# weiguangzhao/PBNet

Hardware: AMD Instinct MI355X
Metric: scenes/sec fwd+cluster (ScanNet ~150k pts/scene) (higher is better)
Workload: dtype bf16; 1 GPU; configs[1]: 1 scene, 161517 pts, 146038 voxels @2cm, 1 rotated copy, full PBNet.forward (MinkUNet34C + grouping + MinkUNet14A mask + MinkUNet34C score); scenes_in_flight_per_gpu=4, scene_seeds=2 (configs[1])

## Files before the change

### include/pbnet_hip.h

```cpp
#ifndef PBNET_HIP_H
#define PBNET_HIP_H

#include <stddef.h>
#include <stdint.h>

#ifdef __cplusplus
extern "C" {
#endif

typedef void* pbn_stream_t;

enum {
    PBN_OK = 0,
    PBN_ERR_ARG = -1,
    PBN_ERR_WORKSPACE = -2,
    PBN_ERR_HIP = -3,
    PBN_ERR_RANGE = -4,
    PBN_ERR_UNSUPPORTED = -5
};

enum { PBN_F32 = 0, PBN_BF16 = 1, PBN_F16 = 2 };

#define PBN_MAX_SCENES 8

// ... 25 lines not shown
                      int capacity, int32_t* unique_index, int32_t* inverse, int32_t* unique_coords, int32_t* n_unique,
                      void* workspace, size_t workspace_bytes, pbn_stream_t stream);

int pbn_coords_stride(const int32_t* fine_coords, const int32_t* n_fine_dev, int n_fine_max, int stride_out,
                      uint64_t* table_keys, int32_t* table_vals, int capacity, int32_t* coarse_coords,
                      int32_t* parent_row, int32_t* child_k, int32_t* nbr_down, int32_t* n_coarse, void* workspace,
                      size_t workspace_bytes, pbn_stream_t stream);

int pbn_kernel_map(const int32_t* out_coords, const int32_t* n_out_dev, int n_out_max, const int32_t* offsets,
                   int n_offsets, const uint64_t* table_keys, const int32_t* table_vals, int capacity, int32_t* nbr,
                   pbn_stream_t stream);

int pbn_kernel_map_cube(const int32_t* out_coords, const int32_t* n_out_dev, int n_out_max, int kernel_size,
                        int tensor_stride, int x_fastest, const uint64_t* table_keys, const int32_t* table_vals,
                        int capacity, int32_t* nbr, pbn_stream_t stream);

int pbn_up_table(const int32_t* parent_row, const int32_t* child_k, const int32_t* n_fine_dev, int n_fine_max,
                 int32_t* nbr_up, pbn_stream_t stream);

int pbn_spconv_forward(const void* in_feat, int ld_in, int n_in, const int32_t* nbr, int n_offsets, const int32_t* row_perm,
                       const int32_t* n_out_dev, int n_out, const void* w_packed, int vecs_per_offset, int n_steps,
                       int cout_padded, const float* scale, const float* shift, const void* residual, int ld_res,
                       int relu, void* out_feat, int ld_out, int dtype, int rows_per_wave, void* workspace,
                       size_t workspace_bytes, pbn_stream_t stream);

int pbn_spconv_forward_dual(const void* in_feat, int ld_in, int n_in, const int32_t* nbr, int n_offsets,
                            const int32_t* n_out_dev, int n_out, const void* w_packed, int vecs_per_offset, int n_steps,
                            int cout_padded, const float* scale, const float* shift, const void* residual, int ld_res,
                            int relu, void* out_feat, int ld_out, int dtype, int rows_per_wave, void* workspace,
                            size_t workspace_bytes, const void* in2_feat, int ld_in2, int n_in2, int vecs_second,
                            pbn_stream_t stream);

int pbn_spconv_family(int n_out, int n_offsets, int vecs_per_offset, int n_steps, int cout_padded, int dtype, int has_map);

int pbn_gather_rows(const void* in, int ld_in_bytes, const int64_t* idx, int n, int row_bytes, void* out,
                    int ld_out_bytes, pbn_stream_t stream);

size_t pbn_segment_pool_workspace_bytes(int n_seg, int channels);
int pbn_segment_pool(const void* feats, int ld, int channels, int dtype, const int32_t* seg_start, int n_seg,
                     float* out_max, float* out_avg, void* workspace, size_t workspace_bytes, pbn_stream_t stream);

int pbn_local_scene_rows(const int32_t* ent_row_start, const int32_t* ent_member_start, const int32_t* ent_scene,
                         const float* ent_weight, int n_ent, int n_rows, const int32_t* member_idx,
                         const int64_t* ins_ind, const float* xyz, float inv_voxel, const void* point_feat, int ld_feat,
                         int channels, const void* sem_score, int ld_sem, const int64_t* sem_pred, int dtype,
                         int64_t* point_idx, int64_t* row_scene, int32_t* coords, void* feat_out, int ld_out,
                         pbn_stream_t stream);
int pbn_gather_pad_rows(const void* in, int ld_in_bytes, int row_bytes, const int64_t* idx, int n, void* out,
                        int ld_out_bytes, pbn_stream_t stream);

int pbn_pack_weight(const float* src, int n_offsets, int dim_a, int dim_b, int flip, int transpose, int dtype,
                    int vecs_per_offset, int n_steps, int cout_padded, void* out, pbn_stream_t stream);

typedef struct pbn_pack_job {
    const float* src;
    void* out;
    int32_t n_offsets, dim_a, dim_b, flip, transpose, cin, cout, cin_p, cout_p, n_steps;
    int32_t reserved[2];
} pbn_pack_job;
int pbn_pack_weights_batch(const pbn_pack_job* jobs, int n_jobs, int max_vectors, int dtype, pbn_stream_t stream);

int pbn_gather_rulebook_rows(const void* in, int ld_in_bytes, int row_bytes, const int32_t* nbr, int n_offsets, int k0,
                             int kc, int n, void* out, pbn_stream_t stream);

size_t pbn_bn_workspace_bytes(int channels);
int pbn_bn_train_forward(const void* x, int ld_x, int n, int channels, int dtype, const float* weight, const float* bias,
// ... 400 lines not shown
```

### pbnet_amd/_native.py

```python
import ctypes
import os

import torch

_HERE = os.path.dirname(os.path.abspath(__file__))
LIB_PATH = os.environ.get("PBNET_HIP_LIB") or os.path.join(_HERE, "libpbnet_hip.so")

_lib = None

c_f32p = ctypes.c_void_p
c_i32p = ctypes.c_void_p
c_vp = ctypes.c_void_p
c_int = ctypes.c_int
c_float = ctypes.c_float
c_size = ctypes.c_size_t

c_i64 = ctypes.c_int64
c_i32 = ctypes.c_int32

DT = {torch.float32: 0, torch.bfloat16: 1, torch.float16: 2}


class CoordsLayout(ctypes.Structure):
    _fields_ = [("counts", c_i64), ("unique_index", c_i64), ("inverse", c_i64),
# ... 74 lines not shown


class ApOverlaps(ctypes.Structure):
    _fields_ = [("n", c_i32), ("_pad", c_i32), ("th", ctypes.c_double * AP_MAX_OVERLAPS)]


class PostBatchLayout(ctypes.Structure):
    _fields_ = [(k, c_i64) for k in ("masks", "counts", "prop_scene", "score", "rows", "pick_rows", "n_rows", "n_pick", "iou",
                                     "votes", "sp_label", "seg", "seg_refined", "counts2", "renumber", "total_bytes")]


SIGNATURES = {
    "pbn_version": (ctypes.c_char_p, []),
    "pbn_last_hip_error": (c_int, []),
    "pbn_cluster_workspace_bytes": (c_size, [c_int, c_int, c_int]),
    "pbn_binary_cluster": (c_int, [c_f32p, c_f32p, c_i32p, c_i32p, c_int, c_int, c_float, c_int, c_float, c_int, c_int,
                                   c_i32p, c_i32p, c_i32p, c_f32p, c_i32p, c_i32p, c_i32p, c_i32p, c_vp, c_size, c_vp]),
    "pbn_get_iou": (c_int, [c_i32p, c_i32p, c_vp, c_i32p, c_f32p, c_int, c_int, c_vp]),
    "pbn_cal_iou_and_masklabel": (c_int, [c_i32p, c_i32p, c_vp, c_i32p, c_f32p, c_int, c_int, c_f32p, c_f32p, c_int,
                                          c_vp]),
    "pbn_hash_capacity": (c_int, [c_int]),
    "pbn_coords_workspace_bytes": (c_size, [c_int]),
    "pbn_coords_unique": (c_int, [c_i32p, c_i32p, c_int, c_vp, c_i32p, c_int, c_i32p, c_i32p, c_i32p, c_i32p, c_vp,
                                  c_size, c_vp]),
    "pbn_coords_stride": (c_int, [c_i32p, c_i32p, c_int, c_int, c_vp, c_i32p, c_int, c_i32p, c_i32p, c_i32p, c_i32p,
                                  c_i32p, c_vp, c_size, c_vp]),
    "pbn_kernel_map": (c_int, [c_i32p, c_i32p, c_int, c_i32p, c_int, c_vp, c_i32p, c_int, c_i32p, c_vp]),
    "pbn_up_table": (c_int, [c_i32p, c_i32p, c_i32p, c_int, c_i32p, c_vp]),
    "pbn_spconv_forward": (c_int, [c_vp, c_int, c_int, c_i32p, c_int, c_i32p, c_i32p, c_int, c_vp, c_int, c_int, c_int,
                                   c_f32p, c_f32p, c_vp, c_int, c_int, c_vp, c_int, c_int, c_int, c_vp, c_size, c_vp]),
    "pbn_spconv_forward_dual": (c_int, [c_vp, c_int, c_int, c_i32p, c_int, c_i32p, c_int, c_vp, c_int, c_int, c_int, c_f32p, c_f32p,
                                        c_vp, c_int, c_int, c_vp, c_int, c_int, c_int, c_vp, c_size, c_vp, c_int, c_int, c_int, c_vp]),
    "pbn_spconv_family": (c_int, [c_int, c_int, c_int, c_int, c_int, c_int, c_int]),
    "pbn_spconv_wgrad_workspace_bytes": (c_size, [c_int, c_int, c_int]),
    "pbn_spconv_wgrad": (c_int, [c_vp, c_int, c_vp, c_int, c_int, c_vp, c_vp, c_i32p, c_i32p, c_int, c_int, c_int, c_int, c_int,
                                 c_f32p, c_vp, c_size, c_vp]),
    "pbn_spconv_wgrad_checked": (c_int, [c_vp, c_int, ctypes.c_longlong, c_vp, c_int, ctypes.c_longlong, c_int, c_vp, c_vp, c_i32p,
                                         c_i32p, c_int, c_int, c_int, c_int, c_int, c_int, c_f32p, c_vp, c_size, c_vp]),
    "pbn_spconv_wgrad_plan": (c_int, [c_int, c_int, c_int, c_int, c_int, c_int, c_int, c_int, c_int, c_int, c_size,
                                      ctypes.POINTER(WgradPlan)]),
    "pbn_gather_rows": (c_int, [c_vp, c_int, c_vp, c_int, c_int, c_vp, c_int, c_vp]),
    "pbn_segment_pool_workspace_bytes": (c_size, [c_int, c_int]),
    "pbn_segment_pool": (c_int, [c_vp, c_int, c_int, c_int, c_i32p, c_int, c_f32p, c_f32p, c_vp, c_size, c_vp]),
    "pbn_local_scene_rows": (c_int, [c_i32p, c_i32p, c_i32p, c_f32p, c_int, c_int, c_i32p, c_vp, c_f32p, c_float, c_vp,
                                     c_int, c_int, c_vp, c_int, c_vp, c_int, c_vp, c_vp, c_i32p, c_vp, c_int, c_vp]),
    "pbn_gather_pad_rows": (c_int, [c_vp, c_int, c_int, c_vp, c_int, c_vp, c_int, c_vp]),
    "pbn_mlp_rows": (c_int, [c_vp, c_int, c_int, c_vp, c_vp, c_int, c_f32p, c_f32p, c_f32p, c_f32p, c_int, c_f32p, c_f32p,
                             c_int, c_int, c_vp, c_int, c_int, c_vp]),
    "pbn_select_blocks": (c_int, [c_int]),
    "pbn_sem_argmax_table": (c_int, [c_vp, c_int, c_int, c_i32p, c_int, c_int, c_int, c_vp, c_vp, c_i32p, c_i32p, c_vp]),
    "pbn_select_points": (c_int, [c_vp, c_int, c_int, c_i32p, c_i32p, c_f32p, c_vp, c_int, c_int, c_vp, c_f32p, c_f32p,
                                  c_i32p, c_vp]),
    "pbn_mask_count": (c_int, [c_vp, c_int, c_float, c_vp, c_int, c_int, c_int, c_i32p, c_i32p, c_vp]),
    "pbn_proposal_rows": (c_int, [c_vp, c_int, c_float, c_vp, c_vp, c_int, c_i32p, c_i32p, c_f32p, c_float, c_float, c_vp,
                                  c_int, c_int, c_int, c_vp, c_vp, c_i32p, c_vp, c_vp]),
    "pbn_post_words": (c_int, [c_int]),
    "pbn_proposal_bitmask": (c_int, [c_vp, c_int, c_int, c_int, c_vp, c_i32p, c_vp]),
    "pbn_mask_iou": (c_int, [c_vp, c_i32p, c_int, c_int, c_i32p, c_f32p, c_vp]),
    "pbn_superpoint_refine": (c_int, [c_vp, c_i32p, c_int, c_int, c_vp, c_int, c_vp, c_i32p, c_vp, c_vp, c_vp, c_i32p,
                                      c_vp]),
    "pbn_bitmask_to_dense": (c_int, [c_vp, c_i32p, c_int, c_int, c_i32p, c_vp]),
    "pbn_post_max_proposals": (c_int, []),
    "pbn_post_select": (c_int, [c_f32p, c_i32p, c_int, c_float, c_int, c_i32p, c_i32p, c_i32p, c_vp]),
    "pbn_mask_iou_dev": (c_int, [c_vp, c_i32p, c_i32p, c_int, c_int, c_i32p, c_f32p, c_vp]),
    "pbn_post_nms": (c_int, [c_f32p, c_i32p, c_i32p, c_int, c_f32p, c_float, c_i32p, c_i32p, c_i32p, c_vp]),
    "pbn_superpoint_refine_dev": (c_int, [c_vp, c_i32p, c_i32p, c_int, c_int, c_vp, c_int, c_vp, c_i32p, c_vp, c_vp, c_vp, c_i32p,
# ... 177 lines not shown
```

### pbnet_amd/csrc/executor.hip

```cpp
#include <cstdlib>
#include "pbn_common.h"
#include "spconv_common.h"
#include "unet_plan.h"

using namespace pbn;

static inline size_t a256(size_t x) { return align_up(x, 256); }

extern "C" size_t pbn_coords_arena_bytes(int n, int want_k5, pbn_coords_layout* L) {
    if (n < 0 || !L) return 0;
    const size_t N = (size_t)(n > 0 ? n : 1);
    const int cap = pbn_hash_capacity(n);
    size_t off = 0;
    auto take = [&](size_t bytes) { size_t o = off; off = a256(off + bytes); return (int64_t)o; };
    L->counts = take(16 * sizeof(int));
    for (int l = 0; l < 5; ++l) { L->capacity[l] = cap; L->keys[l] = take((size_t)cap * 8); }
    for (int l = 0; l < 4; ++l) L->nbr_down[l] = take(N * 8 * 4);
    for (int l = 0; l < 5; ++l) L->vals[l] = take((size_t)cap * 4);
    const int64_t fill_end = (int64_t)off;
    (void)fill_end;
    L->unique_index = take(N * 4);
    L->inverse = take(N * 4);
    for (int l = 0; l < 5; ++l) {
        L->coords[l] = take(N * 16);
// ... 169 lines not shown
}

static NextWeights next_weights(const pbn_unet_op& q, int n_bufs, const MapTables& T, const int32_t* n_rows, const PlanArena& B,
                                int dtype, int mode) {
    if (!op_index_ok(q.in_buf, q.res_buf, q.out_buf, q.level_in, q.level_out, n_bufs) || !q.w) return {};
    const OpTables m = op_tables(q.map_kind, q.level_in, q.level_out, T);
    const ConvArgs nx = shape_args(n_rows[q.level_out], m.K, q.vpo, q.n_steps, q.cout_p, m.fwd != nullptr,
                                   (unsigned)((unsigned long long)q.n_steps * (q.cout_p / 16) * 1024ull),
                                   (unsigned)((unsigned long long)n_rows[q.level_in] * B.ld(q.in_buf) * esize(dtype)));
    LaunchDesc d;
    describe_launch(nx, dtype, &d);
    return {q.w, q.n_steps, q.cout_p / 16, d.wave_family ? d.nt : 0, (mode == 1 && d.wmajor) ? d.groups : 0};
}

static int unet_forward_impl(const pbn_unet_op* ops, int n_ops, const pbn_unet_buf* bufs, int n_bufs,
                             const int32_t* n_rows, const void* input, int ld_input, const int32_t* const* k3,
                             const int32_t* k5, const int32_t* const* down, const int32_t* const* up, void* arena,
                             size_t arena_bytes, int dtype, void* splitk_ws, size_t splitk_bytes, pbn_stream_t stream,
                             hipEvent_t* events, const int32_t* n_rows_dev = nullptr, const int32_t* rows_expected = nullptr) {
    if (!ops || !bufs || !n_rows || !input || !arena || n_ops < 1 || n_bufs < 2 || n_bufs > 512) return PBN_ERR_ARG;
    int64_t offs[512];
    if (pbn_unet_arena_bytes(bufs, n_bufs, n_rows, dtype, offs) > arena_bytes) return PBN_ERR_WORKSPACE;
    static const int pf_env = getenv("PBN_CONV_PREFETCH") ? atoi(getenv("PBN_CONV_PREFETCH")) : 0;
    const PlanArena B(arena, offs, bufs, input, ld_input, esize(dtype));
    const MapTables T{k3, k5, down, up};
    for (int i = 0; i < n_ops; ++i) {
        const pbn_unet_op& o = ops[i];
        if (!op_index_ok(o.in_buf, o.res_buf, o.out_buf, o.level_in, o.level_out, n_bufs)) return PBN_ERR_ARG;
        const OpTables m = op_tables(o.map_kind, o.level_in, o.level_out, T);
        if (!m.ok) return PBN_ERR_ARG;
        const bool dual = o.in2_buf >= 0;
        ConvHints hints;
        if (rows_expected && n_rows_dev) hints.rows_expected = rows_expected[o.level_out];
        if (pf_env && i + 1 < n_ops) hints.next = next_weights(ops[i + 1], n_bufs, T, n_rows, B, dtype, pf_env);
        if (events) PBN_HIP_CHECK(hipEventRecord(events[2 * i], (hipStream_t)stream));
        if (o.in2_buf >= n_bufs) return PBN_ERR_ARG;
        const int rc = spconv_launch({.in_feat = B.at(o.in_buf, o.in_col), .ld_in = B.ld(o.in_buf), .n_in = n_rows[o.level_in],
                                      .nbr = m.fwd, .n_offsets = m.K,
                                      .n_out_dev = n_rows_dev ? n_rows_dev + o.level_out : nullptr, .n_out = n_rows[o.level_out],
                                      .w_packed = o.w, .vecs_per_offset = o.vpo, .n_steps = o.n_steps, .cout_padded = o.cout_p,
                                      .scale = o.scale, .shift = o.shift,
                                      .residual = o.res_buf >= 0 ? B.at(o.res_buf, o.res_col) : nullptr,
                                      .ld_res = o.res_buf >= 0 ? B.ld(o.res_buf) : 0, .relu = o.relu,
                                      .out_feat = B.at(o.out_buf, o.out_col), .ld_out = B.ld(o.out_buf), .dtype = dtype,
                                      .workspace = splitk_ws, .workspace_bytes = splitk_bytes,
                                      .in2_feat = dual ? B.at(o.in2_buf, o.in2_col) : nullptr, .ld_in2 = dual ? B.ld(o.in2_buf) : 0,
                                      .n_in2 = dual ? n_rows[o.level_out] : 0, .vecs_second = dual ? o.vpo2 : 0},
                                     hints, (hipStream_t)stream);
        if (rc != PBN_OK) return rc;
        if (events) PBN_HIP_CHECK(hipEventRecord(events[2 * i + 1], (hipStream_t)stream));
    }
    return PBN_OK;
}

extern "C" int pbn_unet_forward(const pbn_unet_op* ops, int n_ops, const pbn_unet_buf* bufs, int n_bufs,
                                const int32_t* n_rows, const void* input, int ld_input, const int32_t* const* k3,
                                const int32_t* k5, const int32_t* const* down, const int32_t* const* up, void* arena,
                                size_t arena_bytes, int dtype, void* splitk_ws, size_t splitk_bytes, pbn_stream_t stream) {
    return unet_forward_impl(ops, n_ops, bufs, n_bufs, n_rows, input, ld_input, k3, k5, down, up, arena, arena_bytes, dtype,
                             splitk_ws, splitk_bytes, stream, nullptr);
}

extern "C" int pbn_unet_forward_dev(const pbn_unet_op* ops, int n_ops, const pbn_unet_buf* bufs, int n_bufs,
                                    const int32_t* n_rows_cap, const int32_t* n_rows_dev, const int32_t* rows_expected,
                                    const void* input, int ld_input, const int32_t* const* k3, const int32_t* k5,
                                    const int32_t* const* down, const int32_t* const* up, void* arena, size_t arena_bytes,
// ... 28 lines not shown
```

### pbnet_amd/csrc/spconv.hip

```cpp
#include <cmath>
#include <cstdlib>
#include "spconv_common.h"

namespace pbn {
namespace {

constexpr int CGMAX = 4;


#define PBN_LDS_ADDR(p) ((unsigned)(uintptr_t)((__attribute__((address_space(3))) void*)(p)))

#ifdef PBN_CONV_TIMING
__device__ unsigned g_conv_timing[4 * 64 * 8 + 8];
#define PBN_STAMP(POS, I)                                                                                             \
    if (timed_ && lane == 0 && (POS) - g_lo < 64)                                                                     \
        s_time[(wave * 64 + ((POS) - g_lo)) * 8 + (I)] = (unsigned)__builtin_readcyclecounter();
#define PBN_TIMING_SKIP_DMA if (a.dbg & 64) continue
#else
#define PBN_STAMP(POS, I)
#define PBN_TIMING_SKIP_DMA
#endif

template <typename T, int NF, int NT, int RING, int NW = 4>
__global__ __launch_bounds__(NW * 64) void k_spconv(const ConvArgs a) {
// ... 441 lines not shown

__global__ __launch_bounds__(256) void k_gather_rows(const uint4* __restrict__ in, const long long* __restrict__ idx,
                                                    int n, int vec_per_row, int ld_in_vec, int ld_out_vec,
                                                    uint4* __restrict__ out) {
    const long long e = (long long)blockIdx.x * 256 + threadIdx.x;
    if (e >= (long long)n * vec_per_row) return;
    const int i = (int)(e / vec_per_row), v = (int)(e % vec_per_row);
    const long long r = idx[i];
    out[(size_t)i * ld_out_vec + v] = r >= 0 ? in[(size_t)r * ld_in_vec + v] : make_uint4(0u, 0u, 0u, 0u);
}

}
}

using namespace pbn;

namespace {

struct Family { int id; bool (*wanted)(const ConvArgs&, int dtype); int (*launch)(const ConvArgs&, int dtype, int cfg, hipStream_t); };

int launch_wave_auto(const ConvArgs& a, int dtype, int, hipStream_t stream) {
    static const int force_cfg = getenv("PBN_WAVE_CFG") ? atoi(getenv("PBN_WAVE_CFG")) : 0;
    return launch_wave(a, dtype, force_cfg, stream);
}

const Family FAMILIES[] = {
#ifdef PBN_EXPERIMENTS
    {3, pc_family_wanted, launch_pc},
#endif
    {2, rs_family_wanted, launch_rs},
    {1, wave_family_wanted, launch_wave_auto},
};

}

int pbn::spconv_launch(const ConvCall& c, const ConvHints& hints, hipStream_t stream) {
    if (c.n_out < 0 || c.n_in < 0 || c.n_offsets < 1 || c.vecs_per_offset < 1 || c.n_steps < 1 || c.cout_padded < 16 || (c.cout_padded & 15))
        return PBN_ERR_ARG;
    if (!(c.vecs_per_offset == 1 || c.vecs_per_offset == 2 || (c.vecs_per_offset & 3) == 0)) return PBN_ERR_ARG;
    const int n_main = (c.n_offsets * c.vecs_per_offset + 3) / 4;
    if (c.in2_feat) {
        if ((c.vecs_per_offset & 3) || c.vecs_second < 4 || (c.vecs_second & 3) || !c.nbr || c.row_perm || c.n_in2 < c.n_out) return PBN_ERR_ARG;
        if (c.n_steps < n_main + (c.vecs_second >> 2) || c.n_steps > n_main + (c.vecs_second >> 2) + 3) return PBN_ERR_ARG;
    } else if (c.n_steps != n_main) return PBN_ERR_ARG;
    if (!c.nbr && c.n_offsets != 1) return PBN_ERR_ARG;
    if (c.n_out == 0) return PBN_OK;
    if (!c.in_feat || !c.w_packed || !c.out_feat) return PBN_ERR_ARG;
    const int dtype = c.dtype, esz = dtype == PBN_F32 ? 4 : 2;
    if ((c.ld_in * esz) % 16 || (c.ld_out * esz) % 8 || (c.residual && (c.ld_res * esz) % 8)) return PBN_ERR_ARG;
    if (((uintptr_t)c.in_feat | (uintptr_t)c.w_packed) & 15) return PBN_ERR_ARG;
    if (c.in2_feat && ((c.ld_in2 * esz) % 16 || ((uintptr_t)c.in2_feat & 15))) return PBN_ERR_ARG;
    const unsigned long long in2_extent = c.in2_feat ? (unsigned long long)c.n_in2 * (unsigned long long)c.ld_in2 * (unsigned long long)esz : 0ull;
    if (in2_extent >= 0x80000000ull) return PBN_ERR_RANGE;
    const unsigned long long in_extent = (unsigned long long)c.n_in * (unsigned long long)c.ld_in * (unsigned long long)esz;
    const unsigned long long w_extent = (unsigned long long)c.n_steps * (unsigned long long)(c.cout_padded / 16) * 1024ull;
    if (in_extent >= 0x80000000ull || w_extent >= 0x80000000ull) return PBN_ERR_RANGE;
    if (!c.nbr && c.n_in < c.n_out) return PBN_ERR_ARG;
    ConvArgs a;
    a.in_bytes = (unsigned)in_extent; a.w_bytes = (unsigned)w_extent;
    a.in = c.in_feat; a.nbr = c.nbr; a.row_perm = c.row_perm; a.n_out_dev = c.n_out_dev; a.w = c.w_packed; a.scale = c.scale;
    a.shift = c.shift; a.residual = c.residual; a.out = c.out_feat; a.ld_in = c.ld_in; a.ld_res = c.ld_res; a.ld_out = c.ld_out;
    a.K = c.n_offsets; a.vpo = c.vecs_per_offset; a.n_steps = c.n_steps; a.ntiles_total = c.cout_padded / 16; a.n_out = c.n_out;
    a.relu = c.relu;
    a.n_sel = (hints.rows_expected > 0 && c.n_out_dev) ? (hints.rows_expected < c.n_out ? hints.rows_expected : c.n_out) : c.n_out;
    a.ksplit = 1; a.partial = nullptr; a.n_out_pad = 0; a.cg = 1; a.wmajor = 0;
    a.in2 = c.in2_feat; a.ld_in2 = c.ld_in2; a.vpo2 = c.vecs_second; a.n_main = n_main; a.in2_bytes = (unsigned)in2_extent;
    a.pf_w = hints.next.w; a.pf_steps = hints.next.steps; a.pf_ntt = hints.next.ntt; a.pf_nt = hints.next.nt; a.pf_groups = hints.next.groups;
    static const int dbg_env = getenv("PBN_CONV_DBG") ? atoi(getenv("PBN_CONV_DBG")) : 0;
    a.dbg = dbg_env;
    int rows_per_wave = c.rows_per_wave;
    if (rows_per_wave >= 10000) {
        const int cfg = rows_per_wave - 10000;
#ifdef PBN_EXPERIMENTS
        if ((cfg % 100000) / 1000 == 3) return launch_pc(a, dtype, (cfg / 100000) * 16, stream);
#endif
        return launch_rs(a, dtype, cfg, stream);
    }
    if (rows_per_wave >= 100) return launch_wave(a, dtype, rows_per_wave, stream);
    if (rows_per_wave == 0)
        for (const Family& f : FAMILIES)
            if (f.wanted(a, dtype)) {
                const int rc = f.launch(a, dtype, 0, stream);
                if (rc != PBN_ERR_UNSUPPORTED) return rc;
            }
    float* ws = reinterpret_cast<float*>(c.workspace);
    if (((uintptr_t)c.workspace) & 15) ws = nullptr;
    if (rows_per_wave != 16 && rows_per_wave != 32 && rows_per_wave != 64) rows_per_wave = (a.n_sel > 64) ? 32 : 16;
    switch (dtype) {
        case PBN_F32: return launch_t<float>(a, rows_per_wave, ws, c.workspace_bytes, stream);
        case PBN_BF16: return launch_t<__hip_bfloat16>(a, rows_per_wave, ws, c.workspace_bytes, stream);
        case PBN_F16: return launch_t<__half>(a, rows_per_wave, ws, c.workspace_bytes, stream);
        default: return PBN_ERR_ARG;
    }
}

extern "C" int pbn_spconv_forward(const void* in_feat, int ld_in, int n_in, const int32_t* nbr, int n_offsets,
                                  const int32_t* row_perm, const int32_t* n_out_dev, int n_out, const void* w_packed,
                                  int vecs_per_offset, int n_steps, int cout_padded, const float* scale,
                                  const float* shift, const void* residual, int ld_res, int relu, void* out_feat,
                                  int ld_out, int dtype, int rows_per_wave, void* workspace, size_t workspace_bytes,
                                  pbn_stream_t stream) {
    return spconv_launch({.in_feat = in_feat, .ld_in = ld_in, .n_in = n_in, .nbr = nbr, .n_offsets = n_offsets, .row_perm = row_perm,
                          .n_out_dev = n_out_dev, .n_out = n_out, .w_packed = w_packed, .vecs_per_offset = vecs_per_offset,
                          .n_steps = n_steps, .cout_padded = cout_padded, .scale = scale, .shift = shift, .residual = residual,
                          .ld_res = ld_res, .relu = relu, .out_feat = out_feat, .ld_out = ld_out, .dtype = dtype,
                          .rows_per_wave = rows_per_wave, .workspace = workspace, .workspace_bytes = workspace_bytes},
                         ConvHints{}, (hipStream_t)stream);
}

extern "C" int pbn_spconv_family(int n_out, int n_offsets, int vecs_per_offset, int n_steps, int cout_padded, int dtype, int has_map) {
    if (n_out < 0 || n_offsets < 1 || vecs_per_offset < 1 || n_steps < 1 || cout_padded < 16 || (cout_padded & 15)) return PBN_ERR_ARG;
    const ConvArgs a = shape_args(n_out, n_offsets, vecs_per_offset, n_steps, cout_padded, has_map != 0, 0, 0);
    for (const Family& f : FAMILIES)
        if (f.wanted(a, dtype)) return f.id;
    return 0;
}

extern "C" int pbn_spconv_forward_dual(const void* in_feat, int ld_in, int n_in, const int32_t* nbr, int n_offsets,
                                       const int32_t* n_out_dev, int n_out, const void* w_packed, int vecs_per_offset,
                                       int n_steps, int cout_padded, const float* scale, const float* shift,
                                       const void* residual, int ld_res, int relu, void* out_feat, int ld_out, int dtype,
                                       int rows_per_wave, void* workspace, size_t workspace_bytes, const void* in2_feat,
                                       int ld_in2, int n_in2, int vecs_second, pbn_stream_t stream) {
    if (!in2_feat) return PBN_ERR_ARG;
    return spconv_launch({.in_feat = in_feat, .ld_in = ld_in, .n_in = n_in, .nbr = nbr, .n_offsets = n_offsets, .n_out_dev = n_out_dev,
                          .n_out = n_out, .w_packed = w_packed, .vecs_per_offset = vecs_per_offset, .n_steps = n_steps,
                          .cout_padded = cout_padded, .scale = scale, .shift = shift, .residual = residual, .ld_res = ld_res,
                          .relu = relu, .out_feat = out_feat, .ld_out = ld_out, .dtype = dtype, .rows_per_wave = rows_per_wave,
                          .workspace = workspace, .workspace_bytes = workspace_bytes, .in2_feat = in2_feat, .ld_in2 = ld_in2,
                          .n_in2 = n_in2, .vecs_second = vecs_second},
                         ConvHints{}, (hipStream_t)stream);
}

#ifdef PBN_CONV_TIMING
extern "C" int pbn_conv_timing_read(unsigned* host) {
    PBN_HIP_CHECK(hipDeviceSynchronize());
    PBN_HIP_CHECK(hipMemcpyFromSymbol(host, HIP_SYMBOL(pbn::g_conv_timing), sizeof(unsigned) * (4 * 64 * 8 + 8)));
    return PBN_OK;
}
#endif
// ... 15 lines not shown
```

### pbnet_amd/csrc/spconv_common.h

```cpp
#pragma once
#include <hip/hip_bf16.h>
#include <hip/hip_fp16.h>
#include "pbn_common.h"

namespace pbn {

typedef float f32x4 __attribute__((ext_vector_type(4)));
typedef unsigned u32x4 __attribute__((ext_vector_type(4)));
typedef int i32x4 __attribute__((ext_vector_type(4)));
typedef __bf16 bf16x8 __attribute__((ext_vector_type(8)));
typedef _Float16 f16x8 __attribute__((ext_vector_type(8)));

struct ConvArgs {
    const void* in;
    const int* nbr;
    const int* row_perm;
    const int* n_out_dev;
    const void* w;
    const float* scale;
    const float* shift;
    const void* residual;
    void* out;
    int ld_in, ld_res, ld_out;
    unsigned in_bytes, w_bytes;
    int K, vpo, n_steps, ntiles_total;
    int n_out, relu;
    int n_sel;
    int ksplit;
    float* partial;
    int n_out_pad;
    int cg;
    int wmajor;
    int dbg;
    const void* in2;
    int ld_in2, vpo2, n_main;
    unsigned in2_bytes;
    const void* pf_w;
    int pf_steps, pf_ntt, pf_nt, pf_groups;
};

struct LaunchDesc { int wave_family, nt, groups, wmajor; };
struct NextWeights { const void* w; int steps, ntt, nt, groups; };
struct ConvCall {
    const void* in_feat; int ld_in; int n_in;
    const int32_t* nbr; int n_offsets;
    const int32_t* row_perm = nullptr; const int32_t* n_out_dev = nullptr; int n_out;
    const void* w_packed; int vecs_per_offset; int n_steps; int cout_padded;
    const float* scale = nullptr; const float* shift = nullptr; const void* residual = nullptr; int ld_res = 0; int relu = 0;
    void* out_feat; int ld_out; int dtype; int rows_per_wave = 0;
    void* workspace = nullptr; size_t workspace_bytes = 0;
    const void* in2_feat = nullptr; int ld_in2 = 0; int n_in2 = 0; int vecs_second = 0;
};
struct ConvHints { int rows_expected = 0; NextWeights next = {}; };
int spconv_launch(const ConvCall& c, const ConvHints& hints, hipStream_t stream);
inline ConvArgs shape_args(int n_sel, int K, int vpo, int n_steps, int cout_p, bool has_map, unsigned w_bytes, unsigned in_bytes) {
    static const int no_neighbour = -1;
    ConvArgs a{};
    a.nbr = has_map ? &no_neighbour : nullptr;
    a.K = K; a.vpo = vpo; a.n_steps = n_steps; a.ntiles_total = cout_p / 16; a.n_out = a.n_sel = n_sel;
    a.w_bytes = w_bytes; a.in_bytes = in_bytes;
    return a;
}

namespace {

template <typename T> struct Tr;
template <> struct Tr<float> { static constexpr int ELEMS = 4; };
template <> struct Tr<__hip_bfloat16> { static constexpr int ELEMS = 8; };
template <> struct Tr<__half> { static constexpr int ELEMS = 8; };

template <typename T>
__device__ __forceinline__ void mfma_step(const u32x4& w, const u32x4& x, f32x4& acc);

template <>
__device__ __forceinline__ void mfma_step<float>(const u32x4& w, const u32x4& x, f32x4& acc) {
    acc = __builtin_amdgcn_mfma_f32_16x16x4f32(__uint_as_float(w[0]), __uint_as_float(x[0]), acc, 0, 0, 0);
    acc = __builtin_amdgcn_mfma_f32_16x16x4f32(__uint_as_float(w[1]), __uint_as_float(x[1]), acc, 0, 0, 0);
    acc = __builtin_amdgcn_mfma_f32_16x16x4f32(__uint_as_float(w[2]), __uint_as_float(x[2]), acc, 0, 0, 0);
    acc = __builtin_amdgcn_mfma_f32_16x16x4f32(__uint_as_float(w[3]), __uint_as_float(x[3]), acc, 0, 0, 0);
}
template <>
__device__ __forceinline__ void mfma_step<__hip_bfloat16>(const u32x4& w, const u32x4& x, f32x4& acc) {
    acc = __builtin_amdgcn_mfma_f32_16x16x32_bf16(__builtin_bit_cast(bf16x8, w), __builtin_bit_cast(bf16x8, x), acc, 0, 0, 0);
}
template <>
__device__ __forceinline__ void mfma_step<__half>(const u32x4& w, const u32x4& x, f32x4& acc) {
// ... 9 lines not shown
    const uint2 v = *reinterpret_cast<const uint2*>(p);
    return f32x4{__uint_as_float(v.x << 16), __uint_as_float(v.x & 0xffff0000u), __uint_as_float(v.y << 16),
                 __uint_as_float(v.y & 0xffff0000u)};
}
template <> __device__ __forceinline__ f32x4 load4<__half>(const __half* p) {
    const uint2 v = *reinterpret_cast<const uint2*>(p);
    const __half2 a = __builtin_bit_cast(__half2, v.x), b = __builtin_bit_cast(__half2, v.y);
    const float2 fa = __half22float2(a), fb = __half22float2(b);
    return f32x4{fa.x, fa.y, fb.x, fb.y};
}
__device__ __forceinline__ unsigned bf16_rne(float f) {
    unsigned u = __float_as_uint(f);
    if ((u & 0x7fffffffu) > 0x7f800000u) return (u >> 16) | 0x40u;
    return (u + 0x7fffu + ((u >> 16) & 1u)) >> 16;
}
template <typename T> __device__ __forceinline__ void store4(T* p, const f32x4& v);
template <> __device__ __forceinline__ void store4<float>(float* p, const f32x4& v) {
    *reinterpret_cast<float4*>(p) = make_float4(v[0], v[1], v[2], v[3]);
}
template <> __device__ __forceinline__ void store4<__hip_bfloat16>(__hip_bfloat16* p, const f32x4& v) {
    uint2 o;
    o.x = bf16_rne(v[0]) | (bf16_rne(v[1]) << 16);
    o.y = bf16_rne(v[2]) | (bf16_rne(v[3]) << 16);
    *reinterpret_cast<uint2*>(p) = o;
}
template <> __device__ __forceinline__ void store4<__half>(__half* p, const f32x4& v) {
    const __half2 a = __floats2half2_rn(v[0], v[1]), b = __floats2half2_rn(v[2], v[3]);
    uint2 o;
    o.x = __builtin_bit_cast(unsigned, a);
    o.y = __builtin_bit_cast(unsigned, b);
    *reinterpret_cast<uint2*>(p) = o;
}

__device__ __forceinline__ void prefetch_drain(u32x4& sink) { asm volatile("s_waitcnt vmcnt(0)" : "+v"(sink)); }
__device__ __forceinline__ u32x4 prefetch_next_weights(const ConvArgs& a, int block, int n_blocks, int tid, int tpb) {
    u32x4 sink = {0u, 0u, 0u, 0u};
    if (!a.pf_w) return sink;
    const int lane = tid & 63, wave = tid >> 6, waves = tpb >> 6;
    int owners = 1, xcd = 0, n_owned = a.pf_ntt / (a.pf_nt > 0 ? a.pf_nt : 1), g0 = 0, gstride = 1;
    if (a.pf_groups > 0) {
        xcd = block & 7;
        owners = 8;
        if (a.pf_groups >= 8) { g0 = xcd; gstride = 8; n_owned = (a.pf_groups - xcd + 7) >> 3; }
        else { g0 = xcd % a.pf_groups; gstride = a.pf_groups; n_owned = 1; }
    } else {
        n_owned = 1;
    }
    const int nt = a.pf_groups > 0 ? a.pf_nt : a.pf_ntt;
    const int rank = a.pf_groups > 0 ? (block >> 3) : block;
    const int nrank = a.pf_groups > 0 ? (n_blocks + 7 - xcd) >> 3 : n_blocks;
    const long long pieces = (long long)a.pf_steps * n_owned * nt;
    const long long per = (pieces + (nrank > 0 ? nrank : 1) - 1) / (nrank > 0 ? nrank : 1);
    const long long lo = (long long)rank * per, hi = lo + per < pieces ? lo + per : pieces;
    (void)owners;
    const unsigned char* base = reinterpret_cast<const unsigned char*>(a.pf_w);
    for (long long q = lo + wave; q < hi; q += waves) {
        const int s = (int)(q / (n_owned * nt));
        const int rem = (int)(q - (long long)s * (n_owned * nt));
        const int gi = rem / nt, t = rem - gi * nt;
        const int tile = (g0 + gi * gstride) * nt + t;
        const u32x4* src = reinterpret_cast<const u32x4*>(base + ((size_t)s * a.pf_ntt + tile) * 1024) + lane;
        asm volatile("global_load_dwordx4 %0, %1, off" : "+v"(sink) : "v"(src) : "memory");
    }
    return sink;
}

__device__ __forceinline__ int xcd_tile(int b, int nt) {
    const int q = nt >> 3, r = nt & 7, xcd = b & 7, idx = b >> 3;
    return (xcd < r ? xcd * (q + 1) : r * (q + 1) + (xcd - r) * q) + idx;
}

}

int launch_wave(const ConvArgs& a, int dtype, int force_cfg, hipStream_t stream);
bool wave_family_wanted(const ConvArgs& a, int dtype);
void describe_launch(const ConvArgs& a, int dtype, LaunchDesc* d);

bool rs_family_wanted(const ConvArgs& a, int dtype);
int launch_rs(const ConvArgs& a, int dtype, int cfg, hipStream_t stream);


#ifdef PBN_EXPERIMENTS
int launch_pc(const ConvArgs& a, int dtype, int rows, hipStream_t stream);
bool pc_family_wanted(const ConvArgs& a, int dtype);
#endif

}
```

### pbnet_amd/csrc/spconv_wave.hip

```cpp
#include <cstdlib>
#include <cstring>
#include "spconv_common.h"

namespace pbn {
namespace {

constexpr unsigned OOB = 0x80000000u;
constexpr unsigned UNIT_NONE = 0xffffu;

constexpr int MAX_DEPTH = 8;

#ifdef PBN_CONV_TIMING
constexpr int WT_BLOCKS = 1024;
__device__ unsigned long long g_wave_timing[WT_BLOCKS * 8 * 8 + 8];
#define PBN_WSTAMP(I)                                                                                                 \
    if (lane == 0 && wt_blk < WT_BLOCKS && wave < 8)                                                                  \
        g_wave_timing[(wt_blk * 8 + wave) * 8 + (I)] = (I) == 7 ? wall_clock64() : __builtin_readcyclecounter();
#else
#define PBN_WSTAMP(I)
#endif
#ifndef PBN_WAVE_DEPTH
#define PBN_WAVE_DEPTH 2
#endif
#ifndef PBN_WAVE_XCOAL
#define PBN_WAVE_XCOAL 1
#endif
constexpr int pipe_depth(int nf, int nt) {
    (void)nf; (void)nt;
    return PBN_WAVE_DEPTH;
}

template <int NF, int NT>
struct Stage {
    u32x4 w[NT];
    u32x4 x[NF];
};

__device__ __forceinline__ void buf_load_asm(u32x4& dst, const i32x4& rs, unsigned voff, unsigned soff) {
    asm volatile("buffer_load_dwordx4 %0, %1, %2, %3 offen" : "+v"(dst) : "v"(voff), "s"(rs), "s"(soff) : "memory");
}

template <typename T>
__device__ __forceinline__ void epilogue_store(const ConvArgs& a, f32x4 v, int orow, int c0) {
    if (a.scale) {
        const float4 sc = *reinterpret_cast<const float4*>(a.scale + c0);
        v[0] *= sc.x; v[1] *= sc.y; v[2] *= sc.z; v[3] *= sc.w;
    }
    if (a.shift) {
        const float4 sh = *reinterpret_cast<const float4*>(a.shift + c0);
        v[0] += sh.x; v[1] += sh.y; v[2] += sh.z; v[3] += sh.w;
    }
    if (a.residual) v += load4<T>(reinterpret_cast<const T*>(a.residual) + (size_t)orow * a.ld_res + c0);
    if (a.relu) {
        v[0] = fmaxf(v[0], 0.f); v[1] = fmaxf(v[1], 0.f); v[2] = fmaxf(v[2], 0.f); v[3] = fmaxf(v[3], 0.f);
    }
    store4<T>(reinterpret_cast<T*>(a.out) + (size_t)orow * a.ld_out + c0, v);
}

#ifndef PBN_WAVE_RED_KB
#define PBN_WAVE_RED_KB 64
#endif
constexpr int ksplit_round_tiles(int kw, int tm, int nt) {
    return (kw * tm * nt * 64 <= PBN_WAVE_RED_KB * 1024) ? nt : (nt < 2 ? nt : 2);
}
constexpr int ksplit_red_pitch(int ntb) { return ntb * 16 + 4; }

struct TileMap { int row_tile, group; bool valid; };
__device__ __forceinline__ TileMap map_block(const ConvArgs& a, int n_row_tiles, int n_groups) {
    TileMap m;
    const int b = blockIdx.x;
    if (!a.wmajor) {
        m.group = b / n_row_tiles;
        m.row_tile = xcd_tile(b - m.group * n_row_tiles, n_row_tiles);
        m.valid = m.group < n_groups;
        return m;
    }
    const int xcd = b & 7, idx = b >> 3;
    if (n_groups >= 8) {
        const int gl = idx / n_row_tiles;
        m.group = xcd + 8 * gl;
        m.row_tile = idx - gl * n_row_tiles;
        m.valid = m.group < n_groups;
    } else {
        const int share = 8 / n_groups;
        m.group = xcd % n_groups;
        m.row_tile = (xcd / n_groups) + share * idx;
        m.valid = m.row_tile < n_row_tiles;
    }
    return m;
// ... 470 lines not shown
```

Before: 381.2 scenes/s.

## Add dedicated transposed-conv kernel for one-neighbour-per-row upsampling layers

Adds a specialised sparse-conv kernel for upsampling layers (map_kind 4), where each fine output row has exactly one parent in the 8-offset kernel map. Rows are bucketed in LDS by the offset they use, so each wave computes only its own offset's GEMM instead of iterating all 8 offsets with mostly empty neighbours. Results are staged through LDS for coalesced stores. The kernel is enabled by default through an executor hint, with an environment switch and a fallback to the existing paths when the shape is unsupported. It adds a new code path, template instantiations and some launch-selection complexity.

```diff
diff --git a/include/pbnet_hip.h b/include/pbnet_hip.h
--- a/include/pbnet_hip.h
+++ b/include/pbnet_hip.h
@@ -81,6 +81,11 @@
                             pbn_stream_t stream);
 
 int pbn_spconv_family(int n_out, int n_offsets, int vecs_per_offset, int n_steps, int cout_padded, int dtype, int has_map);
+
+int pbn_spconv_forward_up(const void* in_feat, int ld_in, int n_in, const int32_t* nbr, int n_offsets, const int32_t* n_out_dev,
+                          int n_out, const void* w_packed, int vecs_per_offset, int n_steps, int cout_padded, const float* scale,
+                          const float* shift, const void* residual, int ld_res, int relu, void* out_feat, int ld_out, int dtype,
+                          int rows_per_wave, void* workspace, size_t workspace_bytes, pbn_stream_t stream);
 
 int pbn_gather_rows(const void* in, int ld_in_bytes, const int64_t* idx, int n, int row_bytes, void* out,
                     int ld_out_bytes, pbn_stream_t stream);
diff --git a/pbnet_amd/_native.py b/pbnet_amd/_native.py
--- a/pbnet_amd/_native.py
+++ b/pbnet_amd/_native.py
@@ -130,6 +130,8 @@
     "pbn_spconv_forward_dual": (c_int, [c_vp, c_int, c_int, c_i32p, c_int, c_i32p, c_int, c_vp, c_int, c_int, c_int, c_f32p, c_f32p,
                                         c_vp, c_int, c_int, c_vp, c_int, c_int, c_int, c_vp, c_size, c_vp, c_int, c_int, c_int, c_vp]),
     "pbn_spconv_family": (c_int, [c_int, c_int, c_int, c_int, c_int, c_int, c_int]),
+    "pbn_spconv_forward_up": (c_int, [c_vp, c_int, c_int, c_i32p, c_int, c_i32p, c_int, c_vp, c_int, c_int, c_int, c_f32p, c_f32p,
+                                      c_vp, c_int, c_int, c_vp, c_int, c_int, c_int, c_vp, c_size, c_vp]),
     "pbn_spconv_wgrad_workspace_bytes": (c_size, [c_int, c_int, c_int]),
     "pbn_spconv_wgrad": (c_int, [c_vp, c_int, c_vp, c_int, c_int, c_vp, c_vp, c_i32p, c_i32p, c_int, c_int, c_int, c_int, c_int,
                                  c_f32p, c_vp, c_size, c_vp]),
diff --git a/pbnet_amd/csrc/executor.hip b/pbnet_amd/csrc/executor.hip
--- a/pbnet_amd/csrc/executor.hip
+++ b/pbnet_amd/csrc/executor.hip
@@ -225,6 +225,7 @@
         const bool dual = o.in2_buf >= 0;
         ConvHints hints;
         if (rows_expected && n_rows_dev) hints.rows_expected = rows_expected[o.level_out];
+        hints.one_pair_per_row = o.map_kind == 4;
         if (pf_env && i + 1 < n_ops) hints.next = next_weights(ops[i + 1], n_bufs, T, n_rows, B, dtype, pf_env);
         if (events) PBN_HIP_CHECK(hipEventRecord(events[2 * i], (hipStream_t)stream));
         if (o.in2_buf >= n_bufs) return PBN_ERR_ARG;
diff --git a/pbnet_amd/csrc/spconv.hip b/pbnet_amd/csrc/spconv.hip
--- a/pbnet_amd/csrc/spconv.hip
+++ b/pbnet_amd/csrc/spconv.hip
@@ -497,9 +497,24 @@
     {1, wave_family_wanted, launch_wave_auto},
 };
 
-}
-
-int pbn::spconv_launch(const ConvCall& c, const ConvHints& hints, hipStream_t stream) {
+int up_order(const ConvArgs& a, int dtype, int rows_per_wave, const void* workspace) {
+    auto ring = [&]() {
+        return (workspace && a.n_sel < 256 * 256) ? 0 : 1;
+    };
+    if (rows_per_wave >= 10000) return 1;
+    if (rows_per_wave >= 2000) return 0;
+    if (rows_per_wave >= 1000) return 2;
+    if (rows_per_wave >= 100) return 1;
+    if (rows_per_wave != 0) return ring();
+    static const int wave_cfg = getenv("PBN_WAVE_CFG") ? atoi(getenv("PBN_WAVE_CFG")) : 0;
+    if (rs_family_wanted(a, dtype)) return 1;
+    if (wave_family_wanted(a, dtype)) return wave_cfg <= 0 ? 2 : up_order(a, dtype, wave_cfg, workspace);
+    return ring();
+}
+
+}
+
+static int spconv_launch_impl(const ConvCall& c, const ConvHints& hints, bool up_only, hipStream_t stream) {
     if (c.n_out < 0 || c.n_in < 0 || c.n_offsets < 1 || c.vecs_per_offset < 1 || c.n_steps < 1 || c.cout_padded < 16 || (c.cout_padded & 15))
         return PBN_ERR_ARG;
     if (!(c.vecs_per_offset == 1 || c.vecs_per_offset == 2 || (c.vecs_per_offset & 3) == 0)) return PBN_ERR_ARG;
@@ -534,6 +549,13 @@
     static const int dbg_env = getenv("PBN_CONV_DBG") ? atoi(getenv("PBN_CONV_DBG")) : 0;
     a.dbg = dbg_env;
     int rows_per_wave = c.rows_per_wave;
+    static const int up_env = getenv("PBN_CONV_UP") ? atoi(getenv("PBN_CONV_UP")) : 1;
+    if (up_only || (hints.one_pair_per_row && up_env && rows_per_wave == 0)) {
+        const void* ws_seen = (((uintptr_t)c.workspace) & 15) ? nullptr : c.workspace;
+        const int order = up_order(a, dtype, rows_per_wave, ws_seen);
+        const int rc = order ? launch_up(a, dtype, order, stream) : PBN_ERR_UNSUPPORTED;
+        if (rc != PBN_ERR_UNSUPPORTED || up_only) return rc;
+    }
     if (rows_per_wave >= 10000) {
         const int cfg = rows_per_wave - 10000;
 #ifdef PBN_EXPERIMENTS
@@ -558,6 +580,8 @@
         default: return PBN_ERR_ARG;
     }
 }
+
+int pbn::spconv_launch(const ConvCall& c, const ConvHints& hints, hipStream_t stream) { return spconv_launch_impl(c, hints, false, stream); }
 
 extern "C" int pbn_spconv_forward(const void* in_feat, int ld_in, int n_in, const int32_t* nbr, int n_offsets,
                                   const int32_t* row_perm, const int32_t* n_out_dev, int n_out, const void* w_packed,
@@ -571,6 +595,20 @@
                           .ld_res = ld_res, .relu = relu, .out_feat = out_feat, .ld_out = ld_out, .dtype = dtype,
                           .rows_per_wave = rows_per_wave, .workspace = workspace, .workspace_bytes = workspace_bytes},
                          ConvHints{}, (hipStream_t)stream);
+}
+
+extern "C" int pbn_spconv_forward_up(const void* in_feat, int ld_in, int n_in, const int32_t* nbr, int n_offsets,
+                                     const int32_t* n_out_dev, int n_out, const void* w_packed, int vecs_per_offset,
+                                     int n_steps, int cout_padded, const float* scale, const float* shift, const void* residual,
+                                     int ld_res, int relu, void* out_feat, int ld_out, int dtype, int rows_per_wave,
+                                     void* workspace, size_t workspace_bytes, pbn_stream_t stream) {
+    if (!nbr || n_offsets != 8) return PBN_ERR_ARG;
+    return spconv_launch_impl({.in_feat = in_feat, .ld_in = ld_in, .n_in = n_in, .nbr = nbr, .n_offsets = n_offsets,
+                               .n_out_dev = n_out_dev, .n_out = n_out, .w_packed = w_packed, .vecs_per_offset = vecs_per_offset,
+                               .n_steps = n_steps, .cout_padded = cout_padded, .scale = scale, .shift = shift, .residual = residual,
+                               .ld_res = ld_res, .relu = relu, .out_feat = out_feat, .ld_out = ld_out, .dtype = dtype,
+                               .rows_per_wave = rows_per_wave, .workspace = workspace, .workspace_bytes = workspace_bytes},
+                              ConvHints{}, true, (hipStream_t)stream);
 }
 
 extern "C" int pbn_spconv_family(int n_out, int n_offsets, int vecs_per_offset, int n_steps, int cout_padded, int dtype, int has_map) {
diff --git a/pbnet_amd/csrc/spconv_common.h b/pbnet_amd/csrc/spconv_common.h
--- a/pbnet_amd/csrc/spconv_common.h
+++ b/pbnet_amd/csrc/spconv_common.h
@@ -51,7 +51,7 @@
     void* workspace = nullptr; size_t workspace_bytes = 0;
     const void* in2_feat = nullptr; int ld_in2 = 0; int n_in2 = 0; int vecs_second = 0;
 };
-struct ConvHints { int rows_expected = 0; NextWeights next = {}; };
+struct ConvHints { int rows_expected = 0; NextWeights next = {}; bool one_pair_per_row = false; };
 int spconv_launch(const ConvCall& c, const ConvHints& hints, hipStream_t stream);
 inline ConvArgs shape_args(int n_sel, int K, int vpo, int n_steps, int cout_p, bool has_map, unsigned w_bytes, unsigned in_bytes) {
     static const int no_neighbour = -1;
@@ -127,6 +127,26 @@
     *reinterpret_cast<uint2*>(p) = o;
 }
 
+template <typename T>
+__device__ __forceinline__ f32x4 epilogue_apply(const ConvArgs& a, f32x4 v, int orow, int c0) {
+    if (a.scale) {
+        const float4 sc = *reinterpret_cast<const float4*>(a.scale + c0);
+        v[0] *= sc.x; v[1] *= sc.y; v[2] *= sc.z; v[3] *= sc.w;
+    }
+    if (a.shift) {
+        const float4 sh = *reinterpret_cast<const float4*>(a.shift + c0);
+        v[0] += sh.x; v[1] += sh.y; v[2] += sh.z; v[3] += sh.w;
+    }
+    if (a.residual) v += load4<T>(reinterpret_cast<const T*>(a.residual) + (size_t)orow * a.ld_res + c0);
+    if (a.relu) {
+        v[0] = fmaxf(v[0], 0.f); v[1] = fmaxf(v[1], 0.f); v[2] = fmaxf(v[2], 0.f); v[3] = fmaxf(v[3], 0.f);
+    }
+    return v;
+}
+template <typename T>
+__device__ __forceinline__ void epilogue_store(const ConvArgs& a, f32x4 v, int orow, int c0) {
+    store4<T>(reinterpret_cast<T*>(a.out) + (size_t)orow * a.ld_out + c0, epilogue_apply<T>(a, v, orow, c0));
+}
 __device__ __forceinline__ void prefetch_drain(u32x4& sink) { asm volatile("s_waitcnt vmcnt(0)" : "+v"(sink)); }
 __device__ __forceinline__ u32x4 prefetch_next_weights(const ConvArgs& a, int block, int n_blocks, int tid, int tpb) {
     u32x4 sink = {0u, 0u, 0u, 0u};
@@ -175,6 +195,8 @@
 int launch_rs(const ConvArgs& a, int dtype, int cfg, hipStream_t stream);
 
 
+int launch_up(const ConvArgs& a, int dtype, int order, hipStream_t stream);
+
 #ifdef PBN_EXPERIMENTS
 int launch_pc(const ConvArgs& a, int dtype, int rows, hipStream_t stream);
 bool pc_family_wanted(const ConvArgs& a, int dtype);
diff --git a/pbnet_amd/csrc/spconv_up.hip b/pbnet_amd/csrc/spconv_up.hip
--- /dev/null
+++ b/pbnet_amd/csrc/spconv_up.hip
@@ -0,0 +1,252 @@
+#include <cstdlib>
+#include "spconv_common.h"
+
+namespace pbn {
+namespace {
+
+constexpr int UP_TPB = 512;
+constexpr int UP_KW = 8;
+
+constexpr bool up_weights_resident(int spo, int nt) { return spo * nt * 4 <= 128; }
+constexpr int up_nf(int esize, int spo, int nt, bool ksplit) {
+    if (!up_weights_resident(spo, nt)) return esize == 4 ? 1 : (ksplit ? 2 : 4);
+    const int nf = (200 - spo * nt * 4) / (spo * 4 + nt * 4 * (ksplit ? 2 : 1));
+    return nf > 4 ? 4 : (nf < 1 ? 1 : nf);
+}
+
+template <typename T, int SPO, int NT, int NF, bool KSPLIT>
+__global__ __launch_bounds__(UP_TPB) void k_spconv_up(const ConvArgs a, const int R) {
+    static_assert(Tr<T>::ELEMS * sizeof(T) == 16, "one gather vector is 16 bytes");
+    static_assert(!KSPLIT || SPO <= UP_KW || SPO % UP_KW == 0, "K-split order: one step per wave, or whole rounds of the 8 waves");
+    constexpr int GS = KSPLIT ? (SPO <= UP_KW ? 1 : SPO / UP_KW) : SPO;
+    constexpr bool WRES = up_weights_resident(SPO, NT);
+    extern __shared__ __attribute__((aligned(16))) unsigned char smem[];
+    int* s_cls = reinterpret_cast<int*>(smem);
+    int* s_src = s_cls + R;
+    int* s_slot = s_src + R;
+
+    const int tid = threadIdx.x, lane = tid & 63;
+    const int wave = __builtin_amdgcn_readfirstlane(tid >> 6);
+    const int g = lane >> 4, rl = lane & 15;
+    const int n = a.n_out_dev ? min(*a.n_out_dev, a.n_out) : a.n_out;
+    const int nt_work = (n + R - 1) / R;
+    if ((int)blockIdx.x >= nt_work) return;
+    const int row0 = xcd_tile(blockIdx.x, nt_work) * R;
+    const int tile0 = blockIdx.y * NT;
+
+    const __amdgpu_buffer_rsrc_t rs_in = __builtin_amdgcn_make_buffer_rsrc(const_cast<void*>(a.in), 0, (int)a.in_bytes, 0x00020000);
+    const __amdgpu_buffer_rsrc_t rs_w = __builtin_amdgcn_make_buffer_rsrc(const_cast<void*>(a.w), 0, (int)a.w_bytes, 0x00020000);
+    constexpr unsigned OOB = 0x80000000u;
+    const unsigned ld_bytes = (unsigned)a.ld_in * (unsigned)sizeof(T);
+    const unsigned wstep = (unsigned)a.ntiles_total * 1024u;
+    const unsigned w0 = ((unsigned)wave * SPO * a.ntiles_total + tile0) * 1024u;
+    const unsigned wlane = (unsigned)lane * 16u;
+    const int b0 = (wave * SPO) & (UP_KW - 1);
+    const int rot = (KSPLIT && GS == 1 && UP_KW - b0 < SPO) ? UP_KW - b0 : 0;
+
+    auto step_of = [&](int i) -> int {
+        if constexpr (!KSPLIT) return i;
+        else if constexpr (GS == 1) { const int j = i + rot; return j >= SPO ? j - SPO : j; }
+        else return i / GS + UP_KW * (i % GS);
+    };
+    u32x4 wr[WRES ? SPO : 1][NT];
+    if constexpr (WRES) {
+#pragma unroll
+        for (int i = 0; i < SPO; ++i)
+#pragma unroll
+            for (int t = 0; t < NT; ++t)
+                wr[i][t] = __builtin_bit_cast(u32x4, __builtin_amdgcn_raw_buffer_load_b128(rs_w, (int)wlane, (int)(w0 + (unsigned)step_of(i) * wstep + (unsigned)t * 1024u), 0));
+    }
+
+    for (int r = tid; r < R; r += UP_TPB) {
+        const int p = row0 + r;
+        int cls = -1, src = -1;
+        if (p < n) {
+            const int4 lo = *reinterpret_cast<const int4*>(a.nbr + (size_t)p * 8);
+            const int4 hi = *reinterpret_cast<const int4*>(a.nbr + (size_t)p * 8 + 4);
+            const int v[8] = {lo.x, lo.y, lo.z, lo.w, hi.x, hi.y, hi.z, hi.w};
+            cls = 8;
+#pragma unroll
+            for (int k = 7; k >= 0; --k)
+                if (v[k] >= 0) { cls = k; src = v[k]; }
+            if (cls == 8) {
+#pragma unroll 1
+                for (int c = 0; c < NT * 4; ++c) epilogue_store<T>(a, f32x4{0.f, 0.f, 0.f, 0.f}, p, tile0 * 16 + c * 4);
+            }
+        }
+        s_cls[r] = cls;
+        s_src[r] = src;
+    }
+    __syncthreads();
+    int* my = s_slot + wave * R;
+    int cnt = 0;
+    for (int base = 0; base < R; base += 64) {
+        const int r = base + lane;
+        const bool m = r < R && s_cls[r] == wave;
+        const unsigned long long b = __ballot(m);
+        if (m) my[cnt + __popcll(b & ((1ull << lane) - 1ull))] = r;
+        cnt += __popcll(b);
+    }
+    const int cnt16 = (cnt + 15) & ~15;
+    if (cnt + lane < cnt16) my[cnt + lane] = -1;
+    __syncthreads();
+
+    if (a.dbg & 2) return;
+    constexpr int ROWB = NT * 16 * (int)sizeof(T);
+    constexpr int VPR = ROWB / 16;
+    constexpr int PITCH = ROWB + 16;
+    unsigned char* stage = smem + sizeof(int) * (size_t)10 * R + (size_t)wave * 16 * PITCH;
+    unsigned char* outb = reinterpret_cast<unsigned char*>(a.out);
+    const bool al16 = ((((size_t)a.ld_out * sizeof(T)) | (uintptr_t)a.out) & 15) == 0;
+#pragma unroll 1
+    for (int fb = 0; fb < cnt16; fb += NF * 16) {
+        int slot[NF];
+        unsigned voff[NF];
+#pragma unroll
+        for (int f = 0; f < NF; ++f) {
+            const int idx = fb + f * 16 + rl;
+            slot[f] = idx < cnt16 ? my[idx] : -1;
+            const int src = slot[f] >= 0 ? s_src[slot[f]] : -1;
+            voff[f] = src >= 0 ? (unsigned)src * ld_bytes + (unsigned)g * 16u : OOB;
+        }
+        f32x4 acc[NF][NT], part[NF][NT];
+        auto close_partial = [&](int i) {
+#pragma unroll
+            for (int f = 0; f < NF; ++f)
+#pragma unroll
+                for (int t = 0; t < NT; ++t) {
+                    if (i / GS == 0) acc[f][t] = part[f][t];
+                    else acc[f][t] += part[f][t];
+                    if constexpr (KSPLIT) asm volatile("" : "+v"(acc[f][t]));
+                }
+        };
+        auto open_partial = [&]() {
+#pragma unroll
+            for (int f = 0; f < NF; ++f)
+#pragma unroll
+                for (int t = 0; t < NT; ++t) part[f][t] = f32x4{0.f, 0.f, 0.f, 0.f};
+        };
+        if constexpr (WRES) {
+            u32x4 x[SPO][NF];
+#pragma unroll
+            for (int i = 0; i < SPO; ++i)
+#pragma unroll
+                for (int f = 0; f < NF; ++f)
+                    x[i][f] = __builtin_bit_cast(u32x4, __builtin_amdgcn_raw_buffer_load_b128(rs_in, (int)voff[f], step_of(i) * 64, 0));
+#pragma unroll
+            for (int i = 0; i < SPO; ++i) {
+                if (i % GS == 0) open_partial();
+#pragma unroll
+                for (int t = 0; t < NT; ++t)
+#pragma unroll
+                    for (int f = 0; f < NF; ++f) mfma_step<T>(wr[i][t], x[i][f], part[f][t]);
+                if (i % GS == GS - 1) close_partial(i);
+            }
+        } else {
+            u32x4 w[2][NT], x[2][NF];
+            auto issue = [&](int i) {
+                const int j = step_of(i);
+#pragma unroll
+                for (int t = 0; t < NT; ++t)
+                    w[i & 1][t] = __builtin_bit_cast(u32x4, __builtin_amdgcn_raw_buffer_load_b128(rs_w, (int)wlane, (int)(w0 + (unsigned)j * wstep + (unsigned)t * 1024u), 0));
+#pragma unroll
+                for (int f = 0; f < NF; ++f)
+                    x[i & 1][f] = __builtin_bit_cast(u32x4, __builtin_amdgcn_raw_buffer_load_b128(rs_in, (int)voff[f], j * 64, 0));
+            };
+            issue(0);
+#pragma unroll
+            for (int i = 0; i < SPO; ++i) {
+                if (i + 1 < SPO) issue(i + 1);
+                __builtin_amdgcn_sched_barrier(0);
+                if (i % GS == 0) open_partial();
+#pragma unroll
+                for (int t = 0; t < NT; ++t)
+#pragma unroll
+                    for (int f = 0; f < NF; ++f) mfma_step<T>(w[i & 1][t], x[i & 1][f], part[f][t]);
+                if (i % GS == GS - 1) close_partial(i);
+                __builtin_amdgcn_sched_barrier(0);
+            }
+        }
+#pragma unroll
+        for (int f = 0; f < NF; ++f) {
+            if (fb + f * 16 >= cnt16) break;
+            const int p = row0 + (slot[f] >= 0 ? slot[f] : 0);
+#pragma unroll
+            for (int t = 0; t < NT; ++t)
+                store4<T>(reinterpret_cast<T*>(stage + rl * PITCH) + t * 16 + g * 4, epilogue_apply<T>(a, acc[f][t], p, (tile0 + t) * 16 + g * 4));
+            __builtin_amdgcn_wave_barrier();
+            if (!(a.dbg & 32)) {
+                for (int e = lane; e < 16 * VPR; e += 64) {
+                    const int row = e / VPR, v = e - row * VPR;
+                    const int sl = my[fb + f * 16 + row];
+                    if (sl < 0) continue;
+                    const u32x4 d = *reinterpret_cast<const u32x4*>(stage + row * PITCH + v * 16);
+                    unsigned char* dst = outb + ((size_t)(row0 + sl) * a.ld_out + tile0 * 16) * sizeof(T) + v * 16;
+                    if (al16) *reinterpret_cast<u32x4*>(dst) = d;
+                    else {
+                        *reinterpret_cast<uint2*>(dst) = make_uint2(d[0], d[1]);
+                        *reinterpret_cast<uint2*>(dst + 8) = make_uint2(d[2], d[3]);
+                    }
+                }
+            }
+            __builtin_amdgcn_wave_barrier();
+        }
+    }
+}
+
+int up_tile_rows(int n_sel, int groups) {
+    static const int force = getenv("PBN_UP_ROWS") ? atoi(getenv("PBN_UP_ROWS")) : 0;
+    if (force >= 64 && force <= 1024) return force & ~63;
+    const int slots = 256 / groups > 0 ? 256 / groups : 1;
+    int r = (int)align_up((size_t)cdiv(n_sel > 0 ? n_sel : 1, slots), 64);
+    return r < 64 ? 64 : (r > 1024 ? 1024 : r);
+}
+
+template <typename T, int SPO, int NT, int NF, bool KSPLIT>
+int launch_up_one(const ConvArgs& a, hipStream_t stream) {
+    const int groups = a.ntiles_total / NT;
+    const int R = up_tile_rows(a.n_sel, groups);
+    const size_t lds = sizeof(int) * (size_t)10 * R + (size_t)8 * 16 * (NT * 16 * sizeof(T) + 16);
+    hipLaunchKernelGGL((k_spconv_up<T, SPO, NT, NF, KSPLIT>), dim3(cdiv(a.n_out, R), groups), dim3(UP_TPB), lds, stream, a, R);
+    PBN_LAUNCH_CHECK();
+    return PBN_OK;
+}
+
+template <typename T, int SPO, bool KSPLIT>
+int launch_up_nt(const ConvArgs& a, hipStream_t stream) {
+    const int ntt = a.ntiles_total;
+    if (ntt % 6 == 0) return launch_up_one<T, SPO, 6, up_nf(sizeof(T), SPO, 6, KSPLIT), KSPLIT>(a, stream);
+    if (ntt % 4 == 0) return launch_up_one<T, SPO, 4, up_nf(sizeof(T), SPO, 4, KSPLIT), KSPLIT>(a, stream);
+    if (ntt % 2 == 0) return launch_up_one<T, SPO, 2, up_nf(sizeof(T), SPO, 2, KSPLIT), KSPLIT>(a, stream);
+    return PBN_ERR_UNSUPPORTED;
+}
+
+template <typename T, bool KSPLIT>
+int launch_up_t(const ConvArgs& a, hipStream_t stream) {
+    const int spo = a.vpo >> 2;
+    if constexpr (sizeof(T) == 4) {
+        if (spo == 6) return launch_up_nt<T, 6, KSPLIT>(a, stream);
+        if (spo == 8) return launch_up_nt<T, 8, KSPLIT>(a, stream);
+        if (spo == 16) return launch_up_nt<T, 16, KSPLIT>(a, stream);
+    } else {
+        if (spo == 3) return launch_up_nt<T, 3, KSPLIT>(a, stream);
+        if (spo == 4) return launch_up_nt<T, 4, KSPLIT>(a, stream);
+        if (spo == 8) return launch_up_nt<T, 8, KSPLIT>(a, stream);
+    }
+    return PBN_ERR_UNSUPPORTED;
+}
+
+}
+
+int launch_up(const ConvArgs& a, int dtype, int order, hipStream_t stream) {
+    if (!a.nbr || a.row_perm || a.in2 || a.K != 8 || (a.vpo & 3) || a.n_steps != 8 * (a.vpo >> 2) || (order != 1 && order != 2))
+        return PBN_ERR_UNSUPPORTED;
+    switch (dtype) {
+        case PBN_F32: return order == 2 ? launch_up_t<float, true>(a, stream) : launch_up_t<float, false>(a, stream);
+        case PBN_BF16: return order == 2 ? launch_up_t<__hip_bfloat16, true>(a, stream) : launch_up_t<__hip_bfloat16, false>(a, stream);
+        case PBN_F16: return order == 2 ? launch_up_t<__half, true>(a, stream) : launch_up_t<__half, false>(a, stream);
+        default: return PBN_ERR_ARG;
+    }
+}
+
+}
diff --git a/pbnet_amd/csrc/spconv_wave.hip b/pbnet_amd/csrc/spconv_wave.hip
--- a/pbnet_amd/csrc/spconv_wave.hip
+++ b/pbnet_amd/csrc/spconv_wave.hip
@@ -38,23 +38,6 @@
 
 __device__ __forceinline__ void buf_load_asm(u32x4& dst, const i32x4& rs, unsigned voff, unsigned soff) {
     asm volatile("buffer_load_dwordx4 %0, %1, %2, %3 offen" : "+v"(dst) : "v"(voff), "s"(rs), "s"(soff) : "memory");
-}
-
-template <typename T>
-__device__ __forceinline__ void epilogue_store(const ConvArgs& a, f32x4 v, int orow, int c0) {
-    if (a.scale) {
-        const float4 sc = *reinterpret_cast<const float4*>(a.scale + c0);
-        v[0] *= sc.x; v[1] *= sc.y; v[2] *= sc.z; v[3] *= sc.w;
-    }
-    if (a.shift) {
-        const float4 sh = *reinterpret_cast<const float4*>(a.shift + c0);
-        v[0] += sh.x; v[1] += sh.y; v[2] += sh.z; v[3] += sh.w;
-    }
-    if (a.residual) v += load4<T>(reinterpret_cast<const T*>(a.residual) + (size_t)orow * a.ld_res + c0);
-    if (a.relu) {
-        v[0] = fmaxf(v[0], 0.f); v[1] = fmaxf(v[1], 0.f); v[2] = fmaxf(v[2], 0.f); v[3] = fmaxf(v[3], 0.f);
-    }
-    store4<T>(reinterpret_cast<T*>(a.out) + (size_t)orow * a.ld_out + c0, v);
 }
 
 #ifndef PBN_WAVE_RED_KB
```

Result: no change. 381.8 scenes/s (median of 6 runs) (+0.2%).
